# rcedgar/urmap

Hardware: AMD Instinct MI355X
Metric: reads/s mapped, 150 bp SE vs hg38, at 1/2/4/8 MI355X; SAM bit-identical (higher is better)
Workload: dtype u8/u64 (fp32 DP cells as the reference)

## Files before the change

### urmap_amd/csrc/kernels.hip

```cpp
#include <algorithm>
#include <cstdlib>

#include "kernels.h"

#include "dev_common.h"
#include "probe_dev.h"
#include "viterbi_dev.h"

namespace urx {

template <int NCH>
__global__ __launch_bounds__(256) void seed_probe_kernel(DevIndex X, const uint8_t *__restrict__ bases,
                                                         const uint64_t *__restrict__ offs, uint32_t n, ProbeOut out) {
	const int lane = threadIdx.x & 63;
	const uint32_t r = blockIdx.x * (blockDim.x >> 6) + (threadIdx.x >> 6);
	if (r >= n) return;
	const uint64_t off = offs[r];
	const uint32_t QL = (uint32_t)(offs[r + 1] - off);
	const uint32_t W = X.W;
	if (QL < W || QL > 64u * NCH) return;
	const uint8_t *q = bases + off;
	probe_read<NCH>(X, q, QL, off, lane, out);
}

// ... 1203 lines not shown
					ok = ok && !S.overlaps_any_hit(s_db - s_qpos);
					const uint64_t m = __ballot(ok);
					if (ok) {
						const int pos = (qhead + qcount + (int)__builtin_amdgcn_mbcnt_hi((uint32_t)(m >> 32), __builtin_amdgcn_mbcnt_lo((uint32_t)m, 0u))) & 127;
						cq_db[pos] = s_db;
						cq_qp[pos] = (uint16_t)(s_qpos | (s_plus ? 0x4000u : 0u) | (g >= totalFirst ? 0x8000u : 0u));
					}
					qcount += __builtin_popcountll(m);
					scanned += 64;
				}
				URX_SYNC();
				const int nb = qcount < 64 ? qcount : 64;
				if (nb == 0) break;
				uint32_t c_qpos = 0, c_db = 0;
				bool c_plus = true, c_second = false;
				const bool c_ok = lane < nb;
				if (c_ok) {
					const int pos = (qhead + lane) & 127;
					c_db = cq_db[pos];
					const uint32_t qp = cq_qp[pos];
					c_qpos = qp & 0x3FFFu; c_plus = (qp & 0x4000u) != 0; c_second = (qp & 0x8000u) != 0;
				}
				qhead = (qhead + nb) & 127; qcount -= nb;
				URX_SYNC();
				bool c_live = c_ok;
				laps(8);
				uint64_t mm[NCH];
#pragma unroll
				for (int c = 0; c < NCH; ++c) mm[c] = 0;
				if (q_other) {
					if (c_live) lane_mismatch_mask<NCH>(g_seq, c_db - c_qpos, sQ2 + (c_plus ? 0 : SW::QMAX), QL, mm);
				} else {
					if (c_live) lane_mismatch_planes<NCH>(g_seqp, c_db - c_qpos, qpl + (c_plus ? 0 : 2 * NCH), QL, mm);
				}
				laps(9);
				int e_kind = 0, e_bst = 0, e_start = 0, e_end = 0, e_pen = 0;
				bool worth = false;
				if (c_live) {
					const int nmis = mismatches_outside_seed<NCH>(mm, (int)c_qpos, W);
					const int floor2 = minhsp > S.best - 4 ? minhsp : S.best - 4;
					worth = -P.mismatch_score * nmis <= S.maxPen || QL - nmis >= floor2;
				}
				if (worth) {
					xdrop_walk_lane<NCH>(mm, (int)c_qpos, W, QL, P.mismatch_score, P.xdrop, S.maxPen, e_bst, e_start, e_end, e_pen);
					if (e_start == 0 && e_end == QL - 1) e_kind = 1;
					else if (e_bst >= minhsp) e_kind = 2;
				}
				laps(10);
				const uint32_t my_dblo = c_db - c_qpos;
				uint64_t todo = __ballot(e_kind != 0 && e_pen <= S.maxPen && !(e_kind == 2 && e_bst < S.best - 4) &&
				                         !S.overlaps_any_hit(my_dblo));
				while (todo) {
					lane = fresh_lane(lane); S.lane = lane;
					const int t = __builtin_ctzll(todo);
					todo &= todo - 1;
					if (rdlane((uint32_t)c_second, t) != 0 && !crossed) {
						crossed = true;
						if (step == 4 && S.best >= minScore3) { done = true; break; }
					}
					const uint32_t dblo = rdlane(my_dblo, t);
					if (S.overlaps_hit(dblo)) continue;
					if (rdlane(e_pen, t) > S.maxPen) continue;
					const bool pl = rdlane((uint32_t)c_plus, t) != 0;
					const int bst = rdlane(e_bst, t);
					const int hc0 = S.hitCount, mp0 = S.maxPen, b0 = S.best;
					if (rdlane(e_kind, t) == 1) {
						S.add_hit(dblo, pl, bst, 0);
						if (step == 1 && bst >= minScore1) { done = true; phase = crossed ? 2 : 1; break; }
					} else {
						const int sp = rdlane(e_start, t), ep = rdlane(e_end, t);
						S.add_hsp((uint32_t)sp, dblo + (uint32_t)sp, pl, (uint32_t)(ep - sp + 1), bst);
						todo &= ~__ballot(e_kind == 2 && my_dblo == dblo && e_bst <= bst);
					}
					if (S.hitCount != hc0 || S.maxPen != mp0 || S.best != b0)
						todo &= __ballot(e_pen <= S.maxPen && !(e_kind == 2 && e_bst < S.best - 4) &&
						                 !(S.hitCount != hc0 && (my_dblo >> 6) == (dblo >> 6)));
				}
				laps(11);
			}

			if (step == 1) {
				lapc(1);
				if (!done) phase = 2;
				step = done ? 5 : 3;
				continue;
			}
			lapc(4);
			if (!done && !crossed && S.best >= minScore3) done = true;
			if (!done) { phase = 5; if (S.best >= minScore4) done = true; }
			if (done) break;
			step = 6;
		}
		lapc(6);
		if (cur_ok && !parked) S.fill_result(res, phase, path_ops, path_used);
		lapc(7);
		if (have_cur && !parked) {
			if constexpr (!OVF) {
				if (res.status & (URMAPX_ST_HSP_OVERFLOW | URMAPX_ST_HIT_OVERFLOW)) {
					if (lane == 0) ovf_list[1 + atomicAdd(ovf_list, 1u)] = r;
				}
			}
			if (lane == 0) results[r] = res;
			if (timing && lane == 0) stats[64 + r] = (uint32_t)((__builtin_amdgcn_s_memtime() - t_read0) >> 4);
		}
		if (!have_next) break;
		have_cur = true; r = rn; off = noff; QL = nQL;
		p3_e = n_e; p3_jb = n_jb; p3_nj = n_nj;
	}
}

__global__ __launch_bounds__(256) void dp_round_lists_kernel(DpWork dp, DpBounds bounds) {
	const uint32_t *const DP_ROUND_LO = bounds.lo;
	constexpr int PER = 16;
	__shared__ uint32_t cnt[DP_ROUNDS], base[DP_ROUNDS];
	const uint32_t made = dp.counters[0];
	const uint32_t njobs = made < dp.jobs_cap ? made : dp.jobs_cap;
	for (uint32_t c0 = blockIdx.x * 256u * PER; c0 < njobs; c0 += gridDim.x * 256u * PER) {
		if (threadIdx.x < DP_ROUNDS) cnt[threadIdx.x] = 0;
		__syncthreads();
		const uint32_t j0 = c0 + threadIdx.x * PER;
		uint16_t kk[PER];
		if (j0 + PER <= njobs) {
			const uint4 a = *reinterpret_cast<const uint4 *>(dp.kidx + j0), b = *reinterpret_cast<const uint4 *>(dp.kidx + j0 + 8);
			const uint32_t w[8] = {a.x, a.y, a.z, a.w, b.x, b.y, b.z, b.w};
#pragma unroll
			for (int i = 0; i < PER; ++i) kk[i] = (uint16_t)(w[i >> 1] >> (16 * (i & 1)));
		} else {
#pragma unroll
			for (int i = 0; i < PER; ++i) kk[i] = j0 + i < njobs ? dp.kidx[j0 + i] : (uint16_t)0xFFFFu;
		}
		uint32_t my[DP_ROUNDS], pos[DP_ROUNDS];
#pragma unroll
		for (int rd = 0; rd < DP_ROUNDS; ++rd) {
			my[rd] = 0;
#pragma unroll
			for (int i = 0; i < PER; ++i) my[rd] += (kk[i] != 0xFFFFu && kk[i] >= DP_ROUND_LO[rd] && kk[i] < DP_ROUND_LO[rd + 1]) ? 1u : 0u;
			pos[rd] = my[rd] ? atomicAdd(&cnt[rd], my[rd]) : 0u;
		}
		__syncthreads();
		if (threadIdx.x < DP_ROUNDS) base[threadIdx.x] = cnt[threadIdx.x] ? atomicAdd(dp.tickets + 8 + threadIdx.x, cnt[threadIdx.x]) : 0u;
		__syncthreads();
#pragma unroll
		for (int rd = 0; rd < DP_ROUNDS; ++rd) {
			uint32_t *out = dp.round_list + (size_t)rd * dp.jobs_cap + base[rd] + pos[rd];
#pragma unroll
			for (int i = 0; i < PER; ++i)
				if (kk[i] != 0xFFFFu && kk[i] >= DP_ROUND_LO[rd] && kk[i] < DP_ROUND_LO[rd + 1]) *out++ = j0 + (uint32_t)i;
		}
		__syncthreads();
	}
}

template <int NCH>
__global__ __launch_bounds__(64) void dp_kernel(DevIndex X, urmapx_params P, const uint8_t *__restrict__ bases,
                                                const uint64_t *__restrict__ offs, DpWork dp, uint8_t *scratch,
                                                size_t scratch_stride, const uint8_t *__restrict__ g_seq, uint32_t klo, uint32_t khi,
                                                uint32_t *ticket, const uint32_t *__restrict__ list, const uint32_t *list_count) {
	constexpr int QMAX = 64 * NCH;
	constexpr int TB_ROWS8 = (QMAX - 24) / 8 + 2;
	__shared__ __attribute__((aligned(16))) uint8_t sQT[QMAX + QMAX + 64];
	uint8_t *const sQ = sQT, *const sT = sQT + QMAX;
	static_assert(QMAX >= 64, "the window lies band_radius + 1 bytes or more inside sQT (viterbi_dev.h: B_LDS)");
	uint32_t *const tb = reinterpret_cast<uint32_t *>(scratch + (size_t)blockIdx.x * scratch_stride +
	                                                  ((WideScratch::bytes(QMAX, QMAX + 64) + 255) & ~(size_t)255));
	__shared__ uint32_t wlds[3 * QMAX];
	__shared__ uint16_t ropsL[OPS_CAP], ropsR[OPS_CAP], cand[URMAPX_MAX_PATH_OPS];
	const int lane = threadIdx.x;
	WideScratch ws;
	ws.carve(scratch + (size_t)blockIdx.x * scratch_stride, QMAX, QMAX + 64);
	const VPar VP(P);
	const int BR = 2 * (int)P.band_radius;
	const uint32_t made = dp.counters[0];
	const uint32_t njobs = made < dp.jobs_cap ? made : dp.jobs_cap;
	auto load_window = [&](uint32_t tlo, int tl) {
		bool gap = false;
		for (int i = lane; i < tl; i += 64) {
			const uint8_t c = g_seq[tlo + i];
			sT[i] = c;
			gap |= (c == '-');
		}
		URX_SYNC();
		return __ballot(gap) != 0;
	};
	uint32_t n_gated = 0;
	uint32_t q_read = 0xFFFFFFFFu;
	bool q_plus = false;
	uint64_t q_off = 0;
	int q_len = 0;
	constexpr uint32_t DP_TILE = 16;
	(void)klo; (void)khi; (void)njobs;
	const uint32_t nlist = *list_count < dp.jobs_cap ? *list_count : dp.jobs_cap;
	uint32_t tile = blockIdx.x * DP_TILE;
	for (bool first = true;; first = false) {
	if (!first) {
		if (tile + DP_TILE >= nlist && tile >= gridDim.x * DP_TILE) break;
		uint32_t t0 = 0;
		if (lane == 0) t0 = atomicAdd(ticket, DP_TILE);
		tile = gridDim.x * DP_TILE + (uint32_t)__builtin_amdgcn_readfirstlane((int)t0);
	}
	if (tile >= nlist) break;
	uint32_t jl = 0xFFFFFFFFu;
	if (lane < (int)DP_TILE && tile + lane < nlist) jl = list ? list[tile + lane] : tile + (uint32_t)lane;
	uint64_t todo = __ballot(jl != 0xFFFFFFFFu);
	while (todo) {
		const uint32_t j = rdlane(jl, __builtin_ctzll(todo));
		todo &= todo - 1;
		const DpJob J = dp.jobs[j];
		if (J.read == 0xFFFFFFFFu) continue;
		{
			const int glen = (int)((J.pk >> PK_LEN_SH) & PK_MASK), gscore = (int)((J.pk >> PK_SCORE_SH) & PK_MASK);
			if (glen - gscore > J.maxpen) {
				if (lane == 0) dp.jobs[j].flags = DPJ_GATED;
				++n_gated;
				continue;
			}
		}
		const uint32_t pk = J.pk, startdb = J.startdb;
		const int startq = (int)(pk & PK_MASK), len = (int)((pk >> PK_LEN_SH) & PK_MASK), hscore = (int)((pk >> PK_SCORE_SH) & PK_MASK);
		const bool plus = (pk >> PK_PLUS_SH) & 1u;
		URX_SYNC();
		if (J.read != q_read || plus != q_plus) {
			if (J.read != q_read) {
				q_off = offs[J.read];
				q_len = (int)(offs[J.read + 1] - q_off);
			}
			const uint8_t *q = bases + q_off;
#pragma unroll
			for (int c = 0; c < NCH; ++c) {
				const int p = 64 * c + lane;
				if (p < q_len) sQ[p] = plus ? q[p] : (uint8_t)comp_char(q[q_len - 1 - p]);
			}
			q_read = J.read; q_plus = plus;
			URX_SYNC();
		}
		const int QL = q_len;
		uint32_t flags = 0, vst_l = 0, vst_r = 0, combinedTLo = startdb;
		int leftScore = 0, rightScore = 0, rtrim = 0;
		int totalPen = len - hscore;
		RevOps RL, RR;
		RL.ops = ropsL; RR.ops = ropsR;
		RL.begin(); RR.begin();
		if (startq > 0) {
			const int leftQL = startq;
			const uint32_t leftTHi = startdb - 1;
			const uint32_t leftTL = (uint32_t)(leftQL + BR);
			if (startdb < (uint32_t)startq || leftTL >= leftTHi) flags |= DPJ_LEFT_FAIL;
			else {
				const uint32_t leftTLo = leftTHi - leftTL + 1;
				if (load_window(leftTLo, (int)leftTL)) flags |= DPJ_LEFT_FAIL;
				else {
					const int allGap = P.gap_open_score + (leftQL - 1) * P.gap_ext_score;
					const int need = leftQL - (J.maxpen - totalPen);
					bool aborted = false;
					leftScore = (int)viterbi_wave<true>(VP, sQ, leftQL, sT, (int)leftTL, true, false, tb, TB_ROWS8, ws, RL, vst_l, lane,
					                                    (float)need, allGap < need ? &aborted : nullptr, wlds, 3 * QMAX);
					if (aborted) { leftScore = need - 1; RL.begin(); vst_l = 0; }
					int nTrimI = 0;
					if (RL.n > 0) {
						const uint32_t lastop = ropsL[RL.n - 1];
						if ((lastop & 3u) == OP_I) { nTrimI = (int)(lastop >> 2); --RL.n; }
					}
					combinedTLo = leftTLo + (uint32_t)nTrimI;
					if (allGap > leftScore) leftScore = allGap;
					totalPen += leftQL - leftScore;
				}
			}
		}
		const int rightQLo = startq + len;
		if (!(flags & DPJ_LEFT_FAIL) && rightQLo < QL) {
			if (totalPen > J.maxpen) flags |= DPJ_RIGHT_SKIPPED;
			else {
				const int rightQL = QL - rightQLo;
				const uint32_t rightTLo = startdb + (uint32_t)len;
				uint32_t rightTHi = rightTLo + (uint32_t)rightQL + (uint32_t)BR;
				if (rightTHi >= X.seqDataSize) rightTHi = X.seqDataSize - 1;
				const uint32_t rightTL = rightTHi - rightTLo + 1;
				if (load_window(rightTLo, (int)rightTL)) flags |= DPJ_RIGHT_FAIL;
				else {
					const int allGap = P.gap_open_score + (rightQL - 1) * P.gap_ext_score;
					const int need = rightQL - (J.maxpen - totalPen);
					bool aborted = false;
					rightScore = (int)viterbi_wave<true>(VP, sQ + rightQLo, rightQL, sT, (int)rightTL, false, true, tb, TB_ROWS8, ws, RR, vst_r, lane,
					                                     (float)need, allGap < need ? &aborted : nullptr, wlds, 3 * QMAX);
					if (aborted) { rightScore = need - 1; RR.begin(); vst_r = 0; flags |= DPJ_RIGHT_ABORTED; }
					if (RR.n > 1 && (ropsR[0] & 3u) == OP_I) rtrim = 1;
					if (allGap > rightScore) rightScore = allGap;
				}
			}
		}
		int nc = 0;
		if (!(flags & (DPJ_LEFT_FAIL | DPJ_RIGHT_FAIL | DPJ_RIGHT_SKIPPED | DPJ_RIGHT_ABORTED))) {
			int cop = -1, clen = 0;
			bool ovf = false;
			auto put = [&](int op, int l) {
				if (l <= 0) return;
				if (op == cop) { clen += l; return; }
				if (clen) { if (nc < URMAPX_MAX_PATH_OPS) { if (lane == 0) cand[nc] = (uint16_t)((clen << 2) | cop); ++nc; } else ovf = true; }
				cop = op; clen = l;
			};
			for (int t = RL.n - 1; t >= 0; --t) { const uint32_t o = ropsL[t]; put((int)(o & 3u), (int)(o >> 2)); }
			put(OP_M, len);
			for (int t = RR.n - 1; t >= rtrim; --t) { const uint32_t o = ropsR[t]; put((int)(o & 3u), (int)(o >> 2)); }
			put(-2, 1);
			if (ovf) { flags |= DPJ_PATH_LONG; nc = 0; }
			URX_SYNC();
			uint16_t *out = dp.ops + (size_t)j * DP_JOB_OPS;
			for (int t = lane; t < nc; t += 64) out[t] = cand[t];
		}
		if (lane == 0) {
			DpJob *o = dp.jobs + j;
			o->combined_tlo = combinedTLo;
			o->left_score = (int16_t)leftScore; o->right_score = (int16_t)rightScore;
			o->nops = (uint8_t)nc; o->flags = (uint8_t)flags; o->vst_l = (uint8_t)vst_l; o->vst_r = (uint8_t)vst_r;
		}
	}
	}
	if (lane == 0 && n_gated) atomicAdd(dp.counters + 3, n_gated);
}

template <int NCH, bool OVF>
__global__ __launch_bounds__(64) __attribute__((amdgpu_waves_per_eu(8, 8))) void finalize_se_kernel(DevIndex X, urmapx_params P, const uint64_t *__restrict__ offs, DpWork dp,
                                                         urmapx_result *__restrict__ results, urmapx_path_op *__restrict__ path_ops,
                                                         uint32_t *path_used, int hsp_lds_cap, uint32_t *ovf_list, uint32_t klo,
                                                         uint32_t khi) {
	using SW = SearchWave<NCH, OVF>;
	__shared__ uint16_t top[URMAPX_MAX_PATH_OPS], cand[URMAPX_MAX_PATH_OPS];
	constexpr int PBUF_OPS = 1024, PEND = 64;
	__shared__ uint16_t pbuf[PBUF_OPS];
	__shared__ uint32_t pend_r[PEND];
	__shared__ urmapx_result pend_res[PEND];
	int pb_used = 0, pb_n = 0;
	const int lane = threadIdx.x;
	auto flush_paths = [&]() {
		if (pb_n == 0) return;
		URX_SYNC();
		uint32_t po = 0;
		if (lane == 0) po = atomicAdd(path_used, (uint32_t)pb_used);
		po = uni(po);
		for (int t = lane; t < pb_used; t += 64) path_ops[po + t] = pbuf[t];
		if (lane < pb_n) {
			urmapx_result rr = pend_res[lane];
			rr.path_off += po;
			results[pend_r[lane]] = rr;
		}
		URX_SYNC();
		pb_used = 0; pb_n = 0;
	};
	SW S(X, P, lane);
	S.W = (int)X.W;
	S.top = top; S.cand = cand;
	S.hsp_lds = (hsp_lds_cap >= 64 && hsp_lds_cap <= HSP_CAP) ? (hsp_lds_cap & ~63) : HSP_CAP;
	S.hit_cap = (hsp_lds_cap >= 64 && hsp_lds_cap <= HSP_CAP) ? S.hsp_lds / 4 : 64 * SE_HITW1;
	S.hit_wsh = (hsp_lds_cap >= 64 && hsp_lds_cap <= HSP_CAP) ? 4 : 6;
	const uint32_t parked = dp.counters[1] < dp.fin_cap ? dp.counters[1] : dp.fin_cap;
	const uint4 *const fin = reinterpret_cast<const uint4 *>(dp.fin_list);
	uint32_t used_block = 0;
	uint4 ent = make_uint4(0u, 0u, 0u, 0u);
	if (blockIdx.x < parked) ent = fin[blockIdx.x];
	for (uint32_t e = blockIdx.x; e < parked; e += gridDim.x) {
		const uint32_t r = uni(ent.x), jb = uni(ent.y), nj = uni(ent.z);
		S.QL = (int)uni(ent.w);
		if (e + gridDim.x < parked) ent = fin[e + gridDim.x];
		if (nj <= klo) continue;
		S.nwords = S.QL - (S.W - 1);
		const uint32_t kend = nj < khi ? nj : khi;
		uint32_t jpk0 = 0;
		uint4 jw0 = make_uint4(0u, 0u, 0u, 0u);
		if (klo + (uint32_t)lane < kend) {
			const uint32_t *jp = reinterpret_cast<const uint32_t *>(dp.jobs + jb + klo + (uint32_t)lane);
			jpk0 = jp[2];
			jw0 = *reinterpret_cast<const uint4 *>(jp + 4);
		}
		URX_SYNC();
		uint32_t *const st = dp.state + (size_t)e * SW::STATE_WORDS;
		const int phase = S.restore_state(st);
		uint32_t used = 0;
		for (uint32_t k0 = klo; k0 < kend; k0 += 64) {
			const uint32_t k = k0 + (uint32_t)lane;
			const uint32_t jpk = jpk0;
			const uint4 jw = jw0;
			jpk0 = 0; jw0 = make_uint4(0u, 0u, 0u, 0u);
			if (k + 64u < kend) {
				const uint32_t *jp = reinterpret_cast<const uint32_t *>(dp.jobs + jb + k + 64u);
				jpk0 = jp[2];
				jw0 = *reinterpret_cast<const uint4 *>(jp + 4);
			}
			const int jstartq = (int)(jpk & PK_MASK), jlen = (int)((jpk >> PK_LEN_SH) & PK_MASK), jhs = (int)((jpk >> PK_SCORE_SH) & PK_MASK);
			const int jpen = jlen - jhs;
			const int jls = (int)(int16_t)(jw.y & 0xFFFFu), jrs = (int)(int16_t)(jw.y >> 16);
			const uint32_t jfl = (jw.z >> 8) & 0xFFu;
			const bool has_l = jstartq > 0, has_r = jstartq + jlen < S.QL;
			const bool raises = (jw.z >> 16) != 0u || (jfl & (DPJ_GATED | DPJ_PATH_LONG)) != 0u;
			const bool dead = (has_l && (jfl & DPJ_LEFT_FAIL)) || (has_r && (jfl & (DPJ_RIGHT_FAIL | DPJ_RIGHT_SKIPPED)));
			const int pen1 = jpen + (has_l ? jstartq - jls : 0);
			const int pen2 = pen1 + (has_r ? (S.QL - (jstartq + jlen)) - jrs : 0);
			const int jscore = jhs + (has_l ? jls : 0) + (has_r ? jrs : 0);
			auto viable = [&]() {
				return k < kend && jpen <= S.maxPen && (raises || (!dead && pen1 <= S.maxPen && pen2 <= S.maxPen && jscore >= S.best - SECONDARY_HIT_MAX_DELTA && jscore >= 10));
			};
			used += (uint32_t)__builtin_popcountll(__ballot(k < kend && jpen <= S.maxPen));
			uint64_t todo = __ballot(viable());
			while (todo) {
				const int t = __builtin_ctzll(todo);
				todo &= todo - 1;
				DpJob J;
				J.read = r; J.startdb = 0; J.maxpen = 0; J.k = 0; J.pad[0] = J.pad[1] = 0;
				J.pk = rdlane(jpk, t);
				J.combined_tlo = rdlane(jw.x, t);
				const uint32_t sc = rdlane(jw.y, t), fl = rdlane(jw.z, t);
				J.left_score = (int16_t)(sc & 0xFFFFu); J.right_score = (int16_t)(sc >> 16);
				J.nops = (uint8_t)(fl & 0xFFu); J.flags = (uint8_t)((fl >> 8) & 0xFFu); J.vst_l = (uint8_t)((fl >> 16) & 0xFFu); J.vst_r = (uint8_t)(fl >> 24);
				const int mp0 = S.maxPen, b0 = S.best;
				S.consume_job(J, dp.ops + (size_t)(jb + k0 + (uint32_t)t) * DP_JOB_OPS);
				if (S.maxPen != mp0 || S.best != b0) todo &= __ballot(viable());
			}
		}
		used_block += used;
		if (nj > khi) {
			URX_SYNC();
			S.park_state(st, phase);
			for (uint32_t k = khi + lane; k < nj; k += 64) dp.jobs[jb + k].maxpen = S.maxPen;
			continue;
		}
		urmapx_result res;
		res.dbpos = 0xFFFFFFFFu; res.seq_index = 0xFFFFFFFFu; res.coord = 0xFFFFFFFFu;
		res.score = 0; res.second = 0; res.mapq = 0; res.plus = 0; res.exit_phase = 0; res.status = 0;
		res.hit_count = 0; res.path_nops = 0; res.path_off = 0;
		if (S.fill_result_core(res, phase)) {
			if (pb_used + S.top_nops > PBUF_OPS || pb_n == PEND) flush_paths();
			URX_SYNC();
			for (int t = lane; t < S.top_nops; t += 64) pbuf[pb_used + t] = top[t];
			res.path_nops = (uint16_t)S.top_nops;
			res.path_off = (uint32_t)pb_used;
			if (lane == 0) { pend_r[pb_n] = r; pend_res[pb_n] = res; }
			pb_used += S.top_nops; ++pb_n;
// ... 379 lines not shown
```

### urmap_amd/csrc/viterbi_dev.h

```cpp
#pragma once
#include "dev_common.h"

namespace urx {

struct WideScratch {
	float *Mr;
	float *Dr;
	uint8_t *TB;
	int la_cap, lb_cap;
	__host__ __device__ static size_t bytes(int la_cap, int lb_cap) {
		return (size_t)2 * (lb_cap + 4) * 4 + (size_t)(la_cap + 1) * (lb_cap + 1);
	}
	__device__ void carve(uint8_t *base, int la, int lb) {
		la_cap = la; lb_cap = lb;
		Mr = reinterpret_cast<float *>(base);
		Dr = Mr + (lb + 4);
		TB = reinterpret_cast<uint8_t *>(Dr + (lb + 4));
	}
};

struct VPar {
	int gap_open_score, gap_ext_score, mismatch_score, band_radius;
	__device__ __forceinline__ VPar(const urmapx_params &P)
	    : gap_open_score(P.gap_open_score), gap_ext_score(P.gap_ext_score), mismatch_score(P.mismatch_score),
	      band_radius((int)P.band_radius) {}
};

struct RevOps {
	uint16_t *ops;
	int cap = OPS_CAP;
	int n;
	int cur_op, cur_len;
	bool overflow;
	__device__ __forceinline__ void begin() { n = 0; cur_op = -1; cur_len = 0; overflow = false; }
	__device__ __forceinline__ void push_run(int op, int len, int lane) {
		do {
			const int piece = len > 16383 ? 16383 : len;
			if (n < cap) {
				if (lane == 0) ops[n] = (uint16_t)((piece << 2) | op);
				++n;
			} else
				overflow = true;
			len -= piece;
		} while (len > 0);
	}
	__device__ __forceinline__ void emit(int op, int lane) {
		if (op == cur_op) ++cur_len;
		else {
			if (cur_len) push_run(cur_op, cur_len, lane);
			cur_op = op; cur_len = 1;
		}
	}
	__device__ __forceinline__ void emit_run(int op, int len, int lane) {
		if (len <= 0) return;
		if (op == cur_op) cur_len += len;
		else {
			if (cur_len) push_run(cur_op, cur_len, lane);
			cur_op = op; cur_len = len;
		}
	}
	__device__ __forceinline__ void end(int lane) {
		if (cur_len) push_run(cur_op, cur_len, lane);
		cur_len = 0; cur_op = -1;
	}
};

__device__ float viterbi_wide(const VPar P, const uint8_t *A, int LA, const uint8_t *B, int LB, bool Left, bool Right,
                              const WideScratch ws, uint32_t *lds, int lds_dwords, RevOps &R, uint32_t &status, int lane);

template <bool B_LDS = false>
__device__ __forceinline__ float viterbi_wave(const VPar P, const uint8_t *A, int LA, const uint8_t *B, int LB, bool Left, bool Right,
                              uint32_t *tb, int tb_rows8, const WideScratch ws, RevOps &R, uint32_t &status, int lane_in,
                              float abort_below = -3.0e38f, bool *aborted = nullptr, uint32_t *wide_lds = nullptr, int wide_lds_dwords = 0) {
	(void)lane_in;
	const int lane = (int)__builtin_amdgcn_mbcnt_hi(~0u, __builtin_amdgcn_mbcnt_lo(~0u, 0u));
	R.begin();
	const float GO = (float)P.gap_open_score, GE = (float)P.gap_ext_score;
	if (LA == 0 || LB == 0) {
		if (LA == 0 && LB == 0) return 0.0f;
		if (LA == 0) { R.emit_run(OP_I, LB, lane); R.end(lane); return (float)(P.gap_open_score + (LB - 1) * P.gap_ext_score); }
		R.emit_run(OP_D, LA, lane); R.end(lane);
		return (float)(P.gap_open_score + (LA - 1) * P.gap_ext_score);
	}
	const int Rad = P.band_radius;
	if constexpr (B_LDS) {
		if ((uint32_t)__builtin_amdgcn_readfirstlane((int)(uint32_t)(uintptr_t)B) < (uint32_t)Rad + 1u) {
			status |= URMAPX_ST_BAND_TOO_WIDE;
			return 0.0f;
		}
	}
	int dlo = min(LA, LB), dhi = max(LA, LB);
	dlo = dlo > Rad ? dlo - Rad : 1;
	dhi += Rad;
	if (dhi > LA + LB - 1) dhi = LA + LB - 1;
	const int ND = dhi - dlo + 1;
	if (ND + 2 > 64 || LB - dlo + 2 > 63 || ((LA + 1 + 7) >> 3) > tb_rows8) {
		if (LA <= ws.la_cap && LB <= ws.lb_cap) {
			if (wide_lds_dwords > 0) return viterbi_wide(P, A, LA, B, LB, Left, Right, ws, wide_lds, wide_lds_dwords, R, status, lane);
			return viterbi_wide(P, A, LA, B, LB, Left, Right, ws, tb, tb_rows8 * 64, R, status, lane);
		}
		status |= URMAPX_ST_BAND_TOO_WIDE;
		return 0.0f;
	}
	const float flane = (float)lane;
	float M = NEG, Dn = NEG;
	uint32_t acc = 0;
	const int jbase = dlo - 1 + lane - LA;
	const bool real = lane >= 1 && lane <= ND;
	auto row_general = [&](int i) {
		const int j = jbase + i;
		const bool active = real && j >= 0 && j < LB;
		const bool semi = (j == LB) && lane >= 1 && lane <= ND + 1;
		const float OpenA = (Left && i == 0) ? 0.0f : GO;
		const float ExtA = (Left && i == 0) ? 0.0f : GE;
		float Mcur = M;
		if (i == 0 && j == 0) Mcur = 0.0f;
		const float D = wave_shl1(Dn, NEG);
		const uint32_t a = A[i];
		const uint32_t b = active ? B[j] : 0u;
		const float v = active ? (Mcur + OpenA) : NEG;
		const float u = v - ExtA * flane;
		const float Pm = wave_prefix_max(u);
		const float I = wave_shr1(Pm, NEG) + ExtA * (flane - 1.0f);
		uint32_t bits = 0;
		if (active) {
			float xM = Mcur;
			if (D > xM) { xM = D; bits = TB_DM; }
			if (I > xM) { xM = I; bits = TB_IM; }
			M = xM + (float)(a == b ? 1 : P.mismatch_score);
			const bool freeB = (j == 0 && Left);
			const float md = Mcur + (freeB ? 0.0f : GO);
			float Dnew = D + (freeB ? 0.0f : GE);
			if (md >= Dnew) { Dnew = md; bits |= TB_MD; }
			Dn = Dnew;
			const float mi = Mcur + OpenA;
			const float Ie = I + ExtA;
			if (mi >= Ie) bits |= TB_MI;
		} else if (semi) {
			const float md = Mcur + GO;
			float Dnew = D + GE;
			if (md >= Dnew) { Dnew = md; bits = TB_MD; }
			Dn = Dnew;
			M = NEG;
		} else if (lane == 0 && j >= 0) {
			bits = TB_IM;
		}
		acc |= bits << (4 * (i & 7));
		if ((i & 7) == 7) { tb[(i >> 3) * 64 + lane] = acc; acc = 0; }
	};
	const float GOl = Left ? 0.0f : GO, GEl = Left ? 0.0f : GE;
	const float MISf = (float)P.mismatch_score;
	const float ONEl = real ? 1.0f : NEG, MISl = real ? MISf : NEG;
	const float el = GE * flane, el1 = GE * (flane - 1.0f);
	const uint32_t LBr = real ? (uint32_t)LB : 0u;
	const int LBs = (lane >= 1 && lane <= ND + 1) ? LB : -(1 << 20);
	const uint32_t bits0c = lane == 0 ? TB_IM : 0u;
	constexpr int RB = 8;
	auto rows_upto = [&](int i0, int n) {
		const int j0 = jbase + i0;
		const uint8_t *Ap = A + i0;
		uint32_t av[RB], bv[RB];
		if constexpr (B_LDS) {
			const uint8_t *Bp = B + j0;
#pragma unroll
			for (int k = 0; k < RB; ++k) { av[k] = Ap[k]; bv[k] = Bp[k]; }
		} else {
#pragma unroll
			for (int k = 0; k < RB; ++k) { av[k] = A[min(i0 + k, LA - 1)]; bv[k] = B[min(max(j0 + k, 0), LB - 1)]; }
		}
		const int sh0 = 4 * (i0 & 7);
		uint32_t word = 0;
#pragma unroll
		for (int k = 0; k < RB; ++k) {
			if (k < n) {
				const int j = j0 + k;
				const bool act = (uint32_t)j < LBr;
				const bool semi = j == LBs;
				const float D = wave_shl1(Dn, NEG);
				const float Mcur = M;
				const float vraw = Mcur + GO;
				const float Pm = wave_prefix_max(vraw - el);
				const float I = wave_shr1(Pm, NEG) + el1;
				uint32_t bits = D > Mcur ? TB_DM : 0u;
				float xM = fmaxf(Mcur, D);
				bits = I > xM ? TB_IM : bits;
				xM = fmaxf(xM, I);
				const float sc = av[k] == bv[k] ? 1.0f : MISf;
				M = xM + (act ? sc : NEG);
				const bool col0 = j == 0;
				const float md = Mcur + (col0 ? GOl : GO);
				const float de = D + (col0 ? GEl : GE);
				const uint32_t bMD = md >= de ? TB_MD : 0u;
				Dn = fmaxf(md, de);
				const uint32_t bMI = vraw >= I + GE ? TB_MI : 0u;
				bits |= bMD | bMI;
				bits = act ? bits : (semi ? bMD : (j >= 0 ? bits0c : 0u));
				word |= bits << (4 * k);
			}
		}
		acc |= word << sh0;
		if (((i0 + n) & 7) == 0) { tb[(i0 >> 3) * 64 + lane] = acc; acc = 0; }
	};
	auto rows_interior = [&](int i0) {
		const int j0 = jbase + i0;
		const uint8_t *Ap = A + i0;
		uint32_t av[RB], bv[RB];
		if constexpr (B_LDS) {
			const uint8_t *Bp = B + j0;
#pragma unroll
			for (int k = 0; k < RB; ++k) { av[k] = Ap[k]; bv[k] = Bp[k]; }
		} else {
#pragma unroll
			for (int k = 0; k < RB; ++k) { av[k] = Ap[k]; bv[k] = B[min(max(j0 + k, 0), LB - 1)]; }
		}
		uint32_t word = 0;
#pragma unroll
		for (int k = 0; k < RB; ++k) {
			const float D = wave_shl1(Dn, NEG);
			const float Mcur = M;
			const float vraw = Mcur + GO;
			const float Pm = wave_prefix_max(vraw - el);
// ... 535 lines not shown
```

Before: 58.21 million.

## Prefetch DP job records, read offsets and reference windows ahead of use

```diff
diff --git a/urmap_amd/csrc/kernels.hip b/urmap_amd/csrc/kernels.hip
--- a/urmap_amd/csrc/kernels.hip
+++ b/urmap_amd/csrc/kernels.hip
@@ -1379,7 +1379,7 @@
 }
 
 template <int NCH>
-__global__ __launch_bounds__(64) void dp_kernel(DevIndex X, urmapx_params P, const uint8_t *__restrict__ bases,
+__global__ __launch_bounds__(64) __attribute__((amdgpu_waves_per_eu(6, 6))) void dp_kernel(DevIndex X, urmapx_params P, const uint8_t *__restrict__ bases,
                                                 const uint64_t *__restrict__ offs, DpWork dp, uint8_t *scratch,
                                                 size_t scratch_stride, const uint8_t *__restrict__ g_seq, uint32_t klo, uint32_t khi,
                                                 uint32_t *ticket, const uint32_t *__restrict__ list, const uint32_t *list_count) {
@@ -1399,7 +1399,54 @@
 	const int BR = 2 * (int)P.band_radius;
 	const uint32_t made = dp.counters[0];
 	const uint32_t njobs = made < dp.jobs_cap ? made : dp.jobs_cap;
-	auto load_window = [&](uint32_t tlo, int tl) {
+	constexpr int WROOM = QMAX + 64;
+	constexpr int WDW = (WROOM + 255) / 256;
+	static_assert(WROOM % 4 == 0 && 256 * WDW >= WROOM, "a window that fits sT fits WDW dwords per lane");
+	constexpr bool EARLY = WDW == 1;
+	auto window_mis = [&](uint32_t tlo) { return (int)(reinterpret_cast<uintptr_t>(g_seq + tlo) & 3); };
+	auto window_early = [&](uint32_t tlo, int tl) { return tl > 0 && window_mis(tlo) + tl <= WROOM; };
+	auto issue_window = [&](uint32_t tlo, int tl, uint32_t (&w)[WDW]) {
+		const int mis = window_mis(tlo), nb = mis + tl;
+		const uint32_t *src = reinterpret_cast<const uint32_t *>(g_seq + tlo - mis);
+#pragma unroll
+		for (int k = 0; k < WDW; ++k) {
+			const int d = 64 * k + lane;
+			w[k] = 4 * d < nb ? src[d] : 0u;
+		}
+	};
+	auto commit_window = [&](uint32_t tlo, int tl, const uint32_t (&w)[WDW]) {
+		const int mis = window_mis(tlo), nb = mis + tl;
+		bool gap = false;
+#pragma unroll
+		for (int k = 0; k < WDW; ++k) {
+			const int d = 64 * k + lane;
+			if (4 * d < nb) {
+				const uint32_t v = w[k];
+				*reinterpret_cast<uint32_t *>(sT + 4 * d) = v;
+				const uint32_t x = v ^ 0x2D2D2D2Du;
+				const uint32_t eq = ~(((x & 0x7F7F7F7Fu) + 0x7F7F7F7Fu) | x | 0x7F7F7F7Fu);
+				const int lo = mis > 4 * d ? mis - 4 * d : 0, hi = nb - 4 * d;
+				const uint32_t in = (hi >= 4 ? 0xFFFFFFFFu : (1u << (8 * hi)) - 1u) & ~((1u << (8 * lo)) - 1u);
+				gap |= (eq & in) != 0;
+			}
+		}
+		URX_SYNC();
+		return __ballot(gap) != 0;
+	};
+	uint32_t *const LW = wlds, *const LREC = wlds + 64 * WDW, *const LOFS = wlds + 64 * WDW + 64;
+	static_assert(64 * WDW + 128 <= 3 * QMAX, "the look-ahead fits the wide path's rows");
+	auto issue_window_lds = [&](uint32_t tlo, int tl) {
+		const int mis = window_mis(tlo), nb = mis + tl;
+		const uint8_t *src = g_seq + tlo - mis;
+		wait_lgkm0();
+#pragma unroll
+		for (int k = 0; k < WDW; ++k)
+			if (256 * k < nb) {
+				const int ob = 256 * k + 4 * lane;
+				glds_dword(src + (ob < nb ? ob : 0), lds_addr(LW + 64 * k));
+			}
+	};
+	auto load_window_late = [&](uint32_t tlo, int tl) {
 		bool gap = false;
 		for (int i = lane; i < tl; i += 64) {
 			const uint8_t c = g_seq[tlo + i];
@@ -1409,11 +1456,17 @@
 		URX_SYNC();
 		return __ballot(gap) != 0;
 	};
+	auto issue_record = [&](uint32_t j) { return lane < 4 ? reinterpret_cast<const uint32_t *>(dp.jobs + j)[lane] : 0u; };
+	auto issue_offsets = [&](uint32_t read) { return lane < 3 ? reinterpret_cast<const uint32_t *>(offs + read)[lane] : 0u; };
+	auto issue_record_lds = [&](uint32_t j) { wait_lgkm0(); glds_dword(reinterpret_cast<const uint32_t *>(dp.jobs + j) + (lane < 4 ? lane : 0), lds_addr(LREC)); };
+	auto issue_offsets_lds = [&](uint32_t read) { wait_lgkm0(); glds_dword(reinterpret_cast<const uint32_t *>(offs + read) + (lane < 3 ? lane : 0), lds_addr(LOFS)); };
 	uint32_t n_gated = 0;
 	uint32_t q_read = 0xFFFFFFFFu;
 	bool q_plus = false;
 	uint64_t q_off = 0;
 	int q_len = 0;
+	bool rec_ahead = false;
+	uint32_t o_read = 0xFFFFFFFFu;
 	constexpr uint32_t DP_TILE = 16;
 	(void)klo; (void)khi; (void)njobs;
 	const uint32_t nlist = *list_count < dp.jobs_cap ? *list_count : dp.jobs_cap;
@@ -1429,38 +1482,83 @@
 	uint32_t jl = 0xFFFFFFFFu;
 	if (lane < (int)DP_TILE && tile + lane < nlist) jl = list ? list[tile + lane] : tile + (uint32_t)lane;
 	uint64_t todo = __ballot(jl != 0xFFFFFFFFu);
+	rec_ahead = false;
 	while (todo) {
 		const uint32_t j = rdlane(jl, __builtin_ctzll(todo));
 		todo &= todo - 1;
-		const DpJob J = dp.jobs[j];
-		if (J.read == 0xFFFFFFFFu) continue;
-		{
-			const int glen = (int)((J.pk >> PK_LEN_SH) & PK_MASK), gscore = (int)((J.pk >> PK_SCORE_SH) & PK_MASK);
-			if (glen - gscore > J.maxpen) {
-				if (lane == 0) dp.jobs[j].flags = DPJ_GATED;
-				++n_gated;
-				continue;
-			}
-		}
-		const uint32_t pk = J.pk, startdb = J.startdb;
+		uint32_t Jread, startdb, pk;
+		int Jmaxpen;
+		if (rec_ahead) {
+			wait_vm0();
+			Jread = uni(LREC[0]); startdb = uni(LREC[1]); pk = uni(LREC[2]); Jmaxpen = (int)uni(LREC[3]);
+		} else {
+			const uint32_t rec = issue_record(j);
+			Jread = rdlane(rec, 0); startdb = rdlane(rec, 1); pk = rdlane(rec, 2); Jmaxpen = (int)rdlane(rec, 3);
+		}
+		rec_ahead = EARLY && todo != 0;
+		if (rec_ahead) issue_record_lds(rdlane(jl, __builtin_ctzll(todo)));
+		if (Jread == 0xFFFFFFFFu) continue;
 		const int startq = (int)(pk & PK_MASK), len = (int)((pk >> PK_LEN_SH) & PK_MASK), hscore = (int)((pk >> PK_SCORE_SH) & PK_MASK);
+		if (len - hscore > Jmaxpen) {
+			if (lane == 0) dp.jobs[j].flags = DPJ_GATED;
+			++n_gated;
+			continue;
+		}
 		const bool plus = (pk >> PK_PLUS_SH) & 1u;
+		uint32_t wL[WDW];
+		const uint32_t leftTHi = startdb - 1, leftTL = (uint32_t)(startq + BR), leftTLo = leftTHi - leftTL + 1;
+		const bool left_ok = startq > 0 && !(startdb < (uint32_t)startq || leftTL >= leftTHi);
+		const bool left_early = EARLY && left_ok && window_early(leftTLo, (int)leftTL);
+		if (left_early) issue_window(leftTLo, (int)leftTL, wL);
+		const bool new_read = Jread != q_read;
+		if (new_read) {
+			if (Jread == o_read) {
+				wait_vm0();
+				const uint32_t o0 = uni(LOFS[0]);
+				q_off = ((uint64_t)uni(LOFS[1]) << 32) | o0;
+				q_len = (int)(uni(LOFS[2]) - o0);
+			} else {
+				const uint32_t ofs = issue_offsets(Jread);
+				q_off = ((uint64_t)rdlane(ofs, 1) << 32) | rdlane(ofs, 0);
+				q_len = (int)(rdlane(ofs, 2) - rdlane(ofs, 0));
+			}
+		}
+		const int QL = q_len;
+		const int rightQLo = startq + len, rightQL = QL - rightQLo;
+		const uint32_t rightTLo = startdb + (uint32_t)len;
+		uint32_t rightTHi = rightTLo + (uint32_t)rightQL + (uint32_t)BR;
+		if (rightTHi >= X.seqDataSize) rightTHi = X.seqDataSize - 1;
+		const uint32_t rightTL = rightTHi - rightTLo + 1;
+		const bool calm = (!left_ok || viterbi_narrow((int)P.band_radius, startq, (int)leftTL, TB_ROWS8)) &&
+		                  (rightQLo >= QL || viterbi_narrow((int)P.band_radius, rightQL, (int)rightTL, TB_ROWS8));
+		const bool right_early = EARLY && calm && rightQLo < QL && window_early(rightTLo, (int)rightTL);
+		if (right_early) issue_window_lds(rightTLo, (int)rightTL);
+		if (EARLY && !calm) { wait_vm0(); rec_ahead = false; o_read = 0xFFFFFFFFu; }
 		URX_SYNC();
-		if (J.read != q_read || plus != q_plus) {
-			if (J.read != q_read) {
-				q_off = offs[J.read];
-				q_len = (int)(offs[J.read + 1] - q_off);
-			}
-			const uint8_t *q = bases + q_off;
-#pragma unroll
-			for (int c = 0; c < NCH; ++c) {
-				const int p = 64 * c + lane;
-				if (p < q_len) sQ[p] = plus ? q[p] : (uint8_t)comp_char(q[q_len - 1 - p]);
-			}
-			q_read = J.read; q_plus = plus;
+		if (new_read || plus != q_plus) {
+			const uintptr_t qa = reinterpret_cast<uintptr_t>(bases + q_off);
+			const int qmis = (int)(qa & 3), nbq = qmis + q_len;
+			const uint32_t *src = reinterpret_cast<const uint32_t *>(qa - qmis);
+			constexpr int QDW = (QMAX / 4 + 63) / 64;
+#pragma unroll
+			for (int c = 0; c < QDW; ++c) {
+				const int d = 64 * c + lane;
+				if (4 * d < q_len) {
+					const int e = qmis + (plus ? 4 * d : q_len - 4 - 4 * d);
+					const int d0 = e >> 2;
+					const uint32_t lo = (d0 >= 0 && 4 * d0 < nbq) ? src[d0] : 0u;
+					const uint32_t hi = (d0 + 1 >= 0 && 4 * (d0 + 1) < nbq) ? src[d0 + 1] : 0u;
+					uint32_t v = (uint32_t)((((uint64_t)hi << 32) | lo) >> (8 * (e & 3)));
+					if (!plus) {
+						v = __builtin_bswap32(v);
+						v = comp_char(v & 0xFFu) | (comp_char((v >> 8) & 0xFFu) << 8) | (comp_char((v >> 16) & 0xFFu) << 16) | (comp_char(v >> 24) << 24);
+					}
+					*reinterpret_cast<uint32_t *>(sQ + 4 * d) = v;
+				}
+			}
+			q_read = Jread; q_plus = plus;
 			URX_SYNC();
 		}
-		const int QL = q_len;
 		uint32_t flags = 0, vst_l = 0, vst_r = 0, combinedTLo = startdb;
 		int leftScore = 0, rightScore = 0, rtrim = 0;
 		int totalPen = len - hscore;
@@ -1469,17 +1567,15 @@
 		RL.begin(); RR.begin();
 		if (startq > 0) {
 			const int leftQL = startq;
-			const uint32_t leftTHi = startdb - 1;
-			const uint32_t leftTL = (uint32_t)(leftQL + BR);
-			if (startdb < (uint32_t)startq || leftTL >= leftTHi) flags |= DPJ_LEFT_FAIL;
+			if (!left_ok) flags |= DPJ_LEFT_FAIL;
 			else {
-				const uint32_t leftTLo = leftTHi - leftTL + 1;
-				if (load_window(leftTLo, (int)leftTL)) flags |= DPJ_LEFT_FAIL;
+				const bool gap = left_early ? commit_window(leftTLo, (int)leftTL, wL) : load_window_late(leftTLo, (int)leftTL);
+				if (gap) flags |= DPJ_LEFT_FAIL;
 				else {
 					const int allGap = P.gap_open_score + (leftQL - 1) * P.gap_ext_score;
-					const int need = leftQL - (J.maxpen - totalPen);
+					const int need = leftQL - (Jmaxpen - totalPen);
 					bool aborted = false;
-					leftScore = (int)viterbi_wave<true>(VP, sQ, leftQL, sT, (int)leftTL, true, false, tb, TB_ROWS8, ws, RL, vst_l, lane,
+					leftScore = (int)viterbi_wave<true>(VP, sQ, leftQL, sT + (left_early ? window_mis(leftTLo) : 0), (int)leftTL, true, false, tb, TB_ROWS8, ws, RL, vst_l, lane,
 					                                    (float)need, allGap < need ? &aborted : nullptr, wlds, 3 * QMAX);
 					if (aborted) { leftScore = need - 1; RL.begin(); vst_l = 0; }
 					int nTrimI = 0;
@@ -1493,21 +1589,29 @@
 				}
 			}
 		}
-		const int rightQLo = startq + len;
+		if (calm && (rec_ahead || right_early)) {
+			wait_vm0();
+			if (rec_ahead) {
+				const uint32_t nread = uni(LREC[0]);
+				if (nread != 0xFFFFFFFFu && nread != q_read && nread != o_read) { issue_offsets_lds(nread); o_read = nread; }
+			}
+		}
 		if (!(flags & DPJ_LEFT_FAIL) && rightQLo < QL) {
-			if (totalPen > J.maxpen) flags |= DPJ_RIGHT_SKIPPED;
+			if (totalPen > Jmaxpen) flags |= DPJ_RIGHT_SKIPPED;
 			else {
-				const int rightQL = QL - rightQLo;
-				const uint32_t rightTLo = startdb + (uint32_t)len;
-				uint32_t rightTHi = rightTLo + (uint32_t)rightQL + (uint32_t)BR;
-				if (rightTHi >= X.seqDataSize) rightTHi = X.seqDataSize - 1;
-				const uint32_t rightTL = rightTHi - rightTLo + 1;
-				if (load_window(rightTLo, (int)rightTL)) flags |= DPJ_RIGHT_FAIL;
+				bool gap;
+				if (right_early) {
+					uint32_t wR[WDW];
+#pragma unroll
+					for (int k = 0; k < WDW; ++k) wR[k] = LW[64 * k + lane];
+					gap = commit_window(rightTLo, (int)rightTL, wR);
+				} else gap = load_window_late(rightTLo, (int)rightTL);
+				if (gap) flags |= DPJ_RIGHT_FAIL;
 				else {
 					const int allGap = P.gap_open_score + (rightQL - 1) * P.gap_ext_score;
-					const int need = rightQL - (J.maxpen - totalPen);
+					const int need = rightQL - (Jmaxpen - totalPen);
 					bool aborted = false;
-					rightScore = (int)viterbi_wave<true>(VP, sQ + rightQLo, rightQL, sT, (int)rightTL, false, true, tb, TB_ROWS8, ws, RR, vst_r, lane,
+					rightScore = (int)viterbi_wave<true>(VP, sQ + rightQLo, rightQL, sT + (right_early ? window_mis(rightTLo) : 0), (int)rightTL, false, true, tb, TB_ROWS8, ws, RR, vst_r, lane,
 					                                     (float)need, allGap < need ? &aborted : nullptr, wlds, 3 * QMAX);
 					if (aborted) { rightScore = need - 1; RR.begin(); vst_r = 0; flags |= DPJ_RIGHT_ABORTED; }
 					if (RR.n > 1 && (ropsR[0] & 3u) == OP_I) rtrim = 1;
diff --git a/urmap_amd/csrc/viterbi_dev.h b/urmap_amd/csrc/viterbi_dev.h
--- a/urmap_amd/csrc/viterbi_dev.h
+++ b/urmap_amd/csrc/viterbi_dev.h
@@ -67,6 +67,17 @@
 
 __device__ float viterbi_wide(const VPar P, const uint8_t *A, int LA, const uint8_t *B, int LB, bool Left, bool Right,
                               const WideScratch ws, uint32_t *lds, int lds_dwords, RevOps &R, uint32_t &status, int lane);
+
+__device__ __forceinline__ bool viterbi_narrow(int Rad, int LA, int LB, int tb_rows8) {
+	if (LA < 0 || LB < 0) return false;
+	if (LA == 0 || LB == 0) return true;
+	int dlo = min(LA, LB), dhi = max(LA, LB);
+	dlo = dlo > Rad ? dlo - Rad : 1;
+	dhi += Rad;
+	if (dhi > LA + LB - 1) dhi = LA + LB - 1;
+	const int ND = dhi - dlo + 1;
+	return !(ND + 2 > 64 || LB - dlo + 2 > 63 || ((LA + 1 + 7) >> 3) > tb_rows8);
+}
 
 template <bool B_LDS = false>
 __device__ __forceinline__ float viterbi_wave(const VPar P, const uint8_t *A, int LA, const uint8_t *B, int LB, bool Left, bool Right,
```

New measurement: 58.18 million. Within noise of the previous version (-0.1%).
